# ruotianluo/ImageCaptioning.pytorch

Measured on AMD Instinct MI355X. Metric: captions/sec/node (UpDown SCST, bs10xsample_n5, 36x2048 feats), higher is better.
Workload: dtype f32; 1 GPU; UpDown SCST (BASELINE configs[2]): per-GPU batch 10 x train_sample_n 5, 36x2048 bottom-up feats, R=E=1000 A=512, vocab 9487, seq_len 20, references packed+cooked + greedy baseline + CIDEr-D + RewardCriterion + BPTT + clip 0.1 + Adam; rotating_batches=4, global_batch=10, seq_len=20, parallelism=dp1 (flat fp32 gradient, no collective)

## Files before the change

### imagecaptioning/pytorch_amd/csrc/attention.hip

```cpp
#include "capmi_common.h"
#include "profile.h"
#include <hip/hip_ext.h>
#include "../../../include/capmi.h"

using namespace capmi;

namespace {

constexpr int NMAX = 8;
constexpr int ATT_THREADS = 512;

__device__ __forceinline__ bool decode_block(int B, int chunks, int &b, int &chunk) {
    const int id = blockIdx.x;
    const int xcd = id & 7, slot = id >> 3;
    b = (slot / chunks) * 8 + xcd;
    chunk = slot % chunks;
    return b < B;
}
inline int grid_blocks(int B, int chunks) { return ((B + 7) / 8) * 8 * chunks; }
inline int pick_rpb(int B, int n) {
    int rpb = (int)(((long long)B * n) / 256);
    if (rpb < 1) rpb = 1;
    if (rpb > n) rpb = n;
    if (rpb > NMAX) rpb = NMAX;
// ... 677 lines not shown

constexpr int KCH = 12;
constexpr int DATT_T = 128;
__global__ __launch_bounds__(DATT_T) void attn_datt_kernel(const float *__restrict__ d_ctx_all, int ld_dctx,
                                                          const float *__restrict__ alpha_all, float *__restrict__ d_att,
                                                          int T, int N, int n, int K, int R) {
    const int b = blockIdx.x, kc = blockIdx.y * KCH;
    const int r = blockIdx.z * DATT_T + threadIdx.x;
    const int total = T * n;
    extern __shared__ float s_al[];
    for (int i = threadIdx.x; i < total * KCH; i += DATT_T) {
        const int row_i = i / KCH, q = i - row_i * KCH;
        const size_t row = (size_t)(row_i / n) * N + b * n + (row_i % n);
        s_al[i] = (kc + q < K) ? alpha_all[row * K + kc + q] : 0.f;
    }
    __syncthreads();
    if (r >= R) return;
    float acc[KCH];
#pragma unroll
    for (int q = 0; q < KCH; ++q) acc[q] = 0.f;
    for (int i0 = 0; i0 < total; i0 += 4) {
        float d[4];
#pragma unroll
        for (int u = 0; u < 4; ++u) {
            const int i = min(i0 + u, total - 1);
            const size_t row = (size_t)(i / n) * N + b * n + (i % n);
            d[u] = (i0 + u < total) ? d_ctx_all[row * ld_dctx + r] : 0.f;
        }
#pragma unroll
        for (int u = 0; u < 4; ++u) {
            const float *al = s_al + min(i0 + u, total - 1) * KCH;
#pragma unroll
            for (int q = 0; q < KCH; ++q) acc[q] += al[q] * d[u];
        }
    }
#pragma unroll
    for (int q = 0; q < KCH; ++q)
        if (kc + q < K) d_att[((size_t)b * K + kc + q) * R + r] = acc[q];
}

template <int KB>
__global__ void attn_dpatt_kernel(const float *__restrict__ att_h_all, const float *__restrict__ d_e_all,
                                  const float *__restrict__ p_att, const float *__restrict__ w,
                                  float *__restrict__ d_p_att, float *__restrict__ d_w, float *__restrict__ dw_part, int T, int N,
                                  int n, int K, int A) {
    const int kblocks = (K + KB - 1) / KB;
    const int b = blockIdx.x / kblocks, k0 = (blockIdx.x % kblocks) * KB;
    const int total = T * n;
    for (int a = threadIdx.x; a < A; a += blockDim.x) {
        float p[KB], acc[KB], accw[KB];
#pragma unroll
        for (int q = 0; q < KB; ++q) {
            p[q] = p_att[((size_t)b * K + min(k0 + q, K - 1)) * A + a];
            acc[q] = accw[q] = 0.f;
        }
        for (int i0 = 0; i0 < total; i0 += 8) {
            float de[8][KB], ah[8];
#pragma unroll
            for (int u = 0; u < 8; ++u) {
                const int i = min(i0 + u, total - 1);
                const size_t row = (size_t)(i / n) * N + b * n + (i % n);
#pragma unroll
                for (int q = 0; q < KB; ++q) de[u][q] = d_e_all[row * K + min(k0 + q, K - 1)];
                ah[u] = att_h_all[row * A + a];
            }
#pragma unroll
            for (int u = 0; u < 8; ++u)
                if (i0 + u < total) {
#pragma unroll
                    for (int q = 0; q < KB; ++q) {
                        const float th = tanh_f(p[q] + ah[u]);
                        acc[q] += de[u][q] * (1.f - th * th);
                        accw[q] += de[u][q] * th;
                    }
                }
        }
#pragma unroll
        for (int q = 0; q < KB; ++q) {
            if (k0 + q >= K) break;
            d_p_att[((size_t)b * K + k0 + q) * A + a] = w[a] * acc[q];
            if (dw_part) dw_part[((size_t)b * K + k0 + q) * A + a] = accw[q];
            else atomicAdd(&d_w[a], accw[q]);
        }
    }
}

__global__ void sum_all_kernel(const float *__restrict__ in, size_t live, size_t slab, size_t count, float *__restrict__ out) {
    __shared__ float scratch[32];
    float s = 0.f;
    const size_t stride = blockDim.x;
    const bool dense = slab == live;
    for (size_t i0 = threadIdx.x; i0 < count; i0 += 8 * stride) {
        float v[8];
#pragma unroll
        for (int u = 0; u < 8; ++u) {
            const size_t i = i0 + u * stride;
            v[u] = i < count ? in[dense ? i : (i / live) * slab + i % live] : 0.f;
        }
#pragma unroll
        for (int u = 0; u < 8; ++u) s += v[u];
    }
    s = block_sum(s, scratch);
    if (threadIdx.x == 0) out[0] = s;
}

}

extern "C" {

static int attention_fwd_launch(const float *att_h, int h_splits, int64_t h_stride, const float *h_bias, float *att_h_out,
                                const float *p_att, const float *att, const float *mask, const float *w, const float *b,
                                float *ctx, float *alpha, int B, int n, int K, int A, int R, const int32_t *row_img, int N,
                                void *stream, unsigned char *pl_ctx = nullptr) {
    if (!att_h || !p_att || !att || !w || !ctx || !alpha || B <= 0 || K <= 0 || A <= 0 || R <= 0) return CAPMI_EINVAL;
    if (row_img ? N <= 0 : n <= 0) return CAPMI_EINVAL;
    if (!row_img) N = B * n;
    if (pl_ctx && N > 64) return CAPMI_EINVAL;
    const size_t lds = ((size_t)NMAX * (A > 1024 ? A : 1024) + (size_t)NMAX * K) * sizeof(float);
    if (lds > 64 * 1024) return CAPMI_EINVAL;
    const double abytes = 4.0 * ((double)B * K * (A + R) + (double)N * (A + R + K));
    const int rpb = row_img ? 1 : pick_rpb_fwd(B, n), chunks = row_img ? 1 : (n + rpb - 1) / rpb;
    hipEvent_t e0, e1;
    static const int env_v2 = capmi::research("CAPMI_ATT_V2", 1);
    const bool al16 = ((reinterpret_cast<uintptr_t>(att_h) | reinterpret_cast<uintptr_t>(p_att) | reinterpret_cast<uintptr_t>(att) |
                        reinterpret_cast<uintptr_t>(w) | reinterpret_cast<uintptr_t>(ctx) | reinterpret_cast<uintptr_t>(h_bias) |
                        reinterpret_cast<uintptr_t>(att_h_out)) & 15) == 0;
    if (env_v2 && al16 && rpb <= 2 && (row_img ? N : grid_blocks(B, chunks)) <= 256 && K <= V2_KMAX && A % 4 == 0 && A >= 4 && A <= 512 && R % 4 == 0 && R >= 4 && R <= 1024 &&
        h_splits <= 16 && (h_stride & 3) == 0) {
        const size_t lds2 = ((size_t)rpb * 1024 + (size_t)rpb * V2_KMAX + (size_t)4 * rpb * 512) * sizeof(float);
        const bool prof = capmi_prof::take_events(CAPMI_PROF_ATTENTION_FWD, &e0, &e1, abytes, (double)N * K * (2.0 * A + 2.0 * R));
        const int gx = row_img ? N : grid_blocks(B, chunks);
        static const int env_cs = capmi::research("CAPMI_ATT_CS", 4);
        const int cs = (env_cs == 2 || env_cs == 4) && gx * env_cs <= 256 ? env_cs : 1;
        const dim3 grid(gx, cs);
#define CAPMI_ATT_V2(NR_, CS_)                                                                                              \
        if (prof) hipExtLaunchKernelGGL((attention_fwd_v2_kernel<NR_, CS_>), grid, dim3(ATT_THREADS), lds2, (hipStream_t)stream, e0, \
                                        e1, 0, att_h, p_att, att, mask, w, b, ctx, alpha, B, n, rpb, chunks, K, A, R, row_img,  \
                                        h_splits, (size_t)h_stride, h_bias, att_h_out, pl_ctx);                                \
        else hipLaunchKernelGGL((attention_fwd_v2_kernel<NR_, CS_>), grid, dim3(ATT_THREADS), lds2, (hipStream_t)stream, att_h, p_att, \
                                att, mask, w, b, ctx, alpha, B, n, rpb, chunks, K, A, R, row_img, h_splits, (size_t)h_stride,   \
                                h_bias, att_h_out, pl_ctx)
        if (rpb == 1) {
            if (cs == 4) { CAPMI_ATT_V2(1, 4); } else if (cs == 2) { CAPMI_ATT_V2(1, 2); } else { CAPMI_ATT_V2(1, 1); }
        } else {
            if (cs == 4) { CAPMI_ATT_V2(2, 4); } else if (cs == 2) { CAPMI_ATT_V2(2, 2); } else { CAPMI_ATT_V2(2, 1); }
        }
#undef CAPMI_ATT_V2
        CAPMI_CHECK_LAUNCH();
        return 0;
    }
    if (capmi_prof::take_events(CAPMI_PROF_ATTENTION_FWD, &e0, &e1, abytes, (double)N * K * (2.0 * A + 2.0 * R)))
        hipExtLaunchKernelGGL(attention_fwd_kernel, dim3(row_img ? N : grid_blocks(B, chunks)), dim3(ATT_THREADS), lds,
                              (hipStream_t)stream, e0, e1, 0, att_h, p_att, att, mask, w, b, ctx, alpha, B, n, rpb, chunks, K,
                              A, R, row_img, h_splits, (size_t)h_stride, h_bias, att_h_out, pl_ctx);
    else
        hipLaunchKernelGGL(attention_fwd_kernel, dim3(row_img ? N : grid_blocks(B, chunks)), dim3(ATT_THREADS), lds,
                           (hipStream_t)stream, att_h, p_att, att, mask, w, b, ctx, alpha, B, n, rpb, chunks, K, A, R, row_img,
                           h_splits, (size_t)h_stride, h_bias, att_h_out, pl_ctx);
    CAPMI_CHECK_LAUNCH();
    return 0;
}

int capmi_attention_fwd(const float *att_h, const float *p_att, const float *att, const float *mask, const float *w,
                        const float *b, float *ctx, float *alpha, int B, int n, int K, int A, int R,
                        const int32_t *row_img, int N, void *stream) {
    return attention_fwd_launch(att_h, 0, 0, nullptr, nullptr, p_att, att, mask, w, b, ctx, alpha, B, n, K, A, R, row_img, N,
// ... 12 lines not shown
int capmi_attention_fwd_partial_pl(const float *h_partial, int h_splits, int64_t h_stride, const float *h_bias,
                                   float *att_h_out, const float *p_att, const float *att, const float *mask, const float *w,
                                   const float *b, float *ctx, float *alpha, int B, int n, int K, int A, int R,
                                   const int32_t *row_img, int N, void *ctx_planes, void *stream) {
    if (h_splits < 1) return CAPMI_EINVAL;
    return attention_fwd_launch(h_partial, h_splits, h_stride, h_bias, att_h_out, p_att, att, mask, w, b, ctx, alpha, B, n, K,
                                A, R, row_img, N, stream, static_cast<unsigned char *>(ctx_planes));
}

static int attention_bwd_launch(const float *d_ctx, int ld_dctx, const float *x_slabs, int x_splits, int64_t x_stride, int x_cols,
                                float *x_out, const float *att_h, const float *alpha, const float *p_att, const float *att,
                                const float *w, float *d_att_h, float *d_e, int B, int n, int K, int A, int R,
                                const int32_t *row_img, int N, void *stream) {
    if (!att_h || !alpha || !p_att || !att || !w || !d_att_h || !d_e || B <= 0) return CAPMI_EINVAL;
    if (row_img ? N <= 0 : n <= 0) return CAPMI_EINVAL;
    if (!row_img) N = B * n;
    const size_t lds = ((size_t)NMAX * ((R + 3) & ~3) + (size_t)NMAX * K) * sizeof(float);
    if (lds > 64 * 1024) return CAPMI_EINVAL;
    const int rpb = row_img ? 1 : pick_rpb(B, n), chunks = row_img ? 1 : (n + rpb - 1) / rpb;
    static const int env_v2 = capmi::research("CAPMI_ATT_BWD_V2", 1);
    if (env_v2 && rpb == 1 && K <= BW2_KMAX && A <= ATT_THREADS && R % 4 == 0 && R <= 1024 &&
        (reinterpret_cast<uintptr_t>(att) & 15) == 0 && (!x_slabs || (x_cols - R) % 4 == 0)) {
        int roles = 1;
        if (x_slabs && x_cols > R) {
            roles = 1 + (x_cols - R + 1023) / 1024;
            if (roles > 4) roles = 4;
        }
        hipLaunchKernelGGL(attention_bwd_v2_kernel, dim3(row_img ? N : grid_blocks(B, chunks), roles), dim3(ATT_THREADS),
                           (size_t)(R + K) * sizeof(float), (hipStream_t)stream, d_ctx, ld_dctx, att_h, alpha, p_att, att, w,
                           d_att_h, d_e, B, n, chunks, K, A, R, row_img, x_slabs, x_splits, (size_t)x_stride, x_cols, x_out);
        CAPMI_CHECK_LAUNCH();
        return 0;
    }
    hipLaunchKernelGGL(attention_bwd_kernel, dim3(row_img ? N : grid_blocks(B, chunks)), dim3(ATT_THREADS), lds,
                       (hipStream_t)stream, d_ctx, ld_dctx, att_h, alpha, p_att, att, w, d_att_h, d_e, B, n, rpb, chunks, K,
                       A, R, row_img, x_slabs, x_splits, (size_t)x_stride, x_cols, x_out);
    CAPMI_CHECK_LAUNCH();
    return 0;
}

int capmi_attention_bwd(const float *d_ctx, int ld_dctx, const float *att_h, const float *alpha, const float *p_att,
                        const float *att, const float *mask, const float *w, float *d_att_h, float *d_e, int B, int n,
                        int K, int A, int R, const int32_t *row_img, int N, void *stream) {
    (void)mask;
    if (!d_ctx || ld_dctx < R) return CAPMI_EINVAL;
    return attention_bwd_launch(d_ctx, ld_dctx, nullptr, 0, 0, 0, nullptr, att_h, alpha, p_att, att, w, d_att_h, d_e, B, n, K, A,
                                R, row_img, N, stream);
}

int capmi_attention_bwd_partial(const float *x_slabs, int x_splits, int64_t x_stride, int x_cols, float *x_out,
                                const float *att_h, const float *alpha, const float *p_att, const float *att,
                                const float *w, float *d_att_h, float *d_e, int B, int n, int K, int A, int R,
                                const int32_t *row_img, int N, void *stream) {
    if (!x_slabs || !x_out || x_splits < 1 || x_cols < R) return CAPMI_EINVAL;
    if ((x_cols & 3) || (x_stride & 3) || ((reinterpret_cast<uintptr_t>(x_slabs) | reinterpret_cast<uintptr_t>(x_out)) & 15)) {
        const int rows = row_img ? N : B * n;
        if (x_stride != (int64_t)rows * x_cols) return CAPMI_EINVAL;
        const int rc = capmi_splitk_reduce(x_slabs, x_splits, x_out, x_cols, rows, x_cols, nullptr, nullptr, nullptr, 1, nullptr, 0,
                                           0, stream);
        if (rc) return rc;
        return attention_bwd_launch(x_out, x_cols, nullptr, 0, 0, 0, nullptr, att_h, alpha, p_att, att, w, d_att_h, d_e, B, n, K, A,
                                    R, row_img, N, stream);
    }
    return attention_bwd_launch(x_out, x_cols, x_slabs, x_splits, x_stride, x_cols, x_out, att_h, alpha, p_att, att, w, d_att_h,
                                d_e, B, n, K, A, R, row_img, N, stream);
}

int capmi_attention_bwd_batched(const float *d_ctx_all, int ld_dctx, const float *att_h_all, const float *alpha_all,
                                const float *d_e_all, const float *p_att, const float *w, float *d_att,
                                float *d_p_att, float *d_w, float *d_b, int T, int B, int n, int N_stride, int K, int A,
                                int R, void *stream) {
    return capmi_attention_bwd_batched_ws(d_ctx_all, ld_dctx, att_h_all, alpha_all, d_e_all, p_att, w, d_att, d_p_att, d_w, d_b, T,
                                          B, n, N_stride, K, A, R, nullptr, stream);
}

int capmi_attention_bwd_batched_ws(const float *d_ctx_all, int ld_dctx, const float *att_h_all, const float *alpha_all,
                                   const float *d_e_all, const float *p_att, const float *w, float *d_att,
                                   float *d_p_att, float *d_w, float *d_b, int T, int B, int n, int N_stride, int K, int A,
                                   int R, float *dw_partial, void *stream) {
    if (!d_ctx_all || !att_h_all || !alpha_all || !d_e_all || !p_att || !w || !d_att || !d_p_att || !d_b) return CAPMI_EINVAL;
    if (!d_w && !dw_partial) return CAPMI_EINVAL;
    hipStream_t st = (hipStream_t)stream;
    const int N = N_stride > 0 ? N_stride : B * n;
    hipLaunchKernelGGL(attn_datt_kernel, dim3(B, (K + KCH - 1) / KCH, (R + DATT_T - 1) / DATT_T), dim3(DATT_T),
                       (size_t)T * n * KCH * sizeof(float), st, d_ctx_all, ld_dctx, alpha_all, d_att, T, N, n, K, R);
    CAPMI_CHECK_LAUNCH();
    if (!dw_partial) {
        hipError_t e = hipMemsetAsync(d_w, 0, (size_t)A * sizeof(float), st);
        if (e != hipSuccess) return (int)e;
    }
    if ((B * ((K + 3) / 4)) >= 512)
        hipLaunchKernelGGL(attn_dpatt_kernel<4>, dim3(B * ((K + 3) / 4)), dim3(A >= 512 ? 512 : 256), 0, st, att_h_all, d_e_all, p_att, w,
                           d_p_att, d_w, dw_partial, T, N, n, K, A);
    else
        hipLaunchKernelGGL(attn_dpatt_kernel<1>, dim3(B * K), dim3(A >= 512 ? 512 : 256), 0, st, att_h_all, d_e_all, p_att, w,
                           d_p_att, d_w, dw_partial, T, N, n, K, A);
    CAPMI_CHECK_LAUNCH();
    hipLaunchKernelGGL(sum_all_kernel, dim3(1), dim3(1024), 0, st, d_e_all, (size_t)B * n * K, (size_t)N * K,
                       (size_t)T * B * n * K, d_b);
    CAPMI_CHECK_LAUNCH();
    return 0;
}

}

#include "host_common.h"

namespace {

constexpr uint64_t TILE_STREAM = 0x74696c65ULL;
constexpr int SSG = 4;

struct TileDrop {
    const float *mask;
    float p, scale;
    uint64_t seed;
    uint64_t row0;
    int on;
};

inline TileDrop tile_drop(const capmi_tile_drop *d) {
    TileDrop t{};
    if (d && (d->mask || d->p > 0.f)) {
        t.on = 1;
        t.mask = d->mask;
        t.p = d->p;
        t.scale = 1.f / (1.f - d->p);
        t.seed = d->seed;
        t.row0 = (uint64_t)d->row0;
    }
    return t;
}

template <int V>
__device__ __forceinline__ void ldv(const float *__restrict__ p, float (&o)[V]) {
    if constexpr (V == 4) {
        const f32x4 t = *reinterpret_cast<const f32x4 *>(p);
        o[0] = t[0]; o[1] = t[1]; o[2] = t[2]; o[3] = t[3];
    } else {
        o[0] = p[0];
    }
}

template <int V>
__device__ __forceinline__ void tile_keep(const TileDrop &td, const Philox &ph, uint64_t row, int kk, int a, int K1, int A,
                                          float (&m)[V]) {
    if (td.mask) {
        ldv<V>(td.mask + (row * K1 + kk) * (uint64_t)A + a, m);
        return;
    }
    const uint64_t idx = ((td.row0 + row) * K1 + kk) * (uint64_t)A + a;
    uint32_t o[4];
    ph.gen(idx >> 2, TILE_STREAM, o);
    if constexpr (V == 4) {
#pragma unroll
        for (int e = 0; e < 4; ++e) m[e] = (u01(o[e]) < td.p) ? 0.f : td.scale;
    } else {
        const uint32_t x = (idx & 2) ? ((idx & 1) ? o[3] : o[2]) : ((idx & 1) ? o[1] : o[0]);
        m[0] = (u01(x) < td.p) ? 0.f : td.scale;
    }
}

__device__ __forceinline__ float slab_sum8(const float *__restrict__ p, int splits, size_t stride) {
    float v = 0.f;
    for (int s0 = 0; s0 < splits; s0 += 8) {
        float part[8];
#pragma unroll
        for (int u = 0; u < 8; ++u) part[u] = (s0 + u < splits) ? p[(size_t)(s0 + u) * stride] : 0.f;
        v += ((part[0] + part[1]) + (part[2] + part[3])) + ((part[4] + part[5]) + (part[6] + part[7]));
    }
    return v;
}

template <int V>
__device__ __forceinline__ void sentinel_scores(const float *__restrict__ pb, const float *__restrict__ w, float bias,
// ... 464 lines not shown
```

### imagecaptioning/pytorch_amd/csrc/capmi_common.h

```cpp
#pragma once
#include <hip/hip_runtime.h>
#include <stdint.h>
#include <stdio.h>
#include <stdlib.h>

#define CAPMI_WAVE 64

#define CAPMI_CHECK_LAUNCH()                      \
    do {                                          \
        hipError_t e__ = hipGetLastError();       \
        if (e__ != hipSuccess) return (int)e__;   \
    } while (0)

typedef float f32x4 __attribute__((ext_vector_type(4)));
typedef float f32x16 __attribute__((ext_vector_type(16)));

namespace capmi {

template <int CTRL>
__device__ __forceinline__ float dpp_f(float v) {
    return __builtin_bit_cast(float, __builtin_amdgcn_update_dpp(0, __builtin_bit_cast(int, v), CTRL, 0xF, 0xF, true));
}
template <int CTRL>
__device__ __forceinline__ int dpp_i(int v) { return __builtin_amdgcn_update_dpp(0, v, CTRL, 0xF, 0xF, true); }
// ... 8 lines not shown
    return (lane_f(v, 0) + lane_f(v, 16)) + (lane_f(v, 32) + lane_f(v, 48));
}
__device__ __forceinline__ float wave_max(float v) {
    v = fmaxf(v, dpp_f<DPP_XOR1>(v));
    v = fmaxf(v, dpp_f<DPP_XOR2>(v));
    v = fmaxf(v, dpp_f<DPP_HALF_MIRROR>(v));
    v = fmaxf(v, dpp_f<DPP_ROW_MIRROR>(v));
    return fmaxf(fmaxf(lane_f(v, 0), lane_f(v, 16)), fmaxf(lane_f(v, 32), lane_f(v, 48)));
}
__device__ __forceinline__ double wave_sum_d(double v) {
#pragma unroll
    for (int o = 32; o > 0; o >>= 1) v += __shfl_xor(v, o, 64);
    return v;
}

__device__ __forceinline__ float block_sum(float v, float *scratch) {
    v = wave_sum(v);
    const int lane = threadIdx.x & 63, wid = threadIdx.x >> 6, nw = (blockDim.x + 63) >> 6;
    __syncthreads();
    if (lane == 0) scratch[wid] = v;
    __syncthreads();
    float r = 0.f;
    for (int i = 0; i < nw; ++i) r += scratch[i];
    return r;
}
__device__ __forceinline__ float block_max(float v, float *scratch) {
    v = wave_max(v);
    const int lane = threadIdx.x & 63, wid = threadIdx.x >> 6, nw = (blockDim.x + 63) >> 6;
    __syncthreads();
    if (lane == 0) scratch[wid] = v;
    __syncthreads();
    float r = scratch[0];
    for (int i = 1; i < nw; ++i) r = fmaxf(r, scratch[i]);
    return r;
}

__device__ __forceinline__ float rcp_f(float x) { return __builtin_amdgcn_rcpf(x); }
__device__ __forceinline__ float tanh_f(float x) {
    const float ax = fabsf(x);
    const float e = __expf(-2.0f * ax);
    const float t = (1.0f - e) * rcp_f(1.0f + e);
    return copysignf(t, x);
}
__device__ __forceinline__ float sigmoid_f(float x) {
    const float e = __expf(-fabsf(x));
    const float s = rcp_f(1.0f + e);
    return x >= 0.f ? s : 1.0f - s;
}

struct Philox {
    uint32_t k0, k1;
    __device__ __forceinline__ Philox(uint64_t seed) : k0((uint32_t)seed), k1((uint32_t)(seed >> 32)) {}
    __device__ __forceinline__ static void round(uint32_t (&c)[4], uint32_t a, uint32_t b) {
        const uint64_t p0 = (uint64_t)0xD2511F53u * c[0];
        const uint64_t p1 = (uint64_t)0xCD9E8D57u * c[2];
        const uint32_t n0 = (uint32_t)(p1 >> 32) ^ c[1] ^ a;
        const uint32_t n1 = (uint32_t)p1;
        const uint32_t n2 = (uint32_t)(p0 >> 32) ^ c[3] ^ b;
        const uint32_t n3 = (uint32_t)p0;
        c[0] = n0; c[1] = n1; c[2] = n2; c[3] = n3;
    }
    __device__ __forceinline__ void gen(uint64_t ctr_lo, uint64_t ctr_hi, uint32_t (&out)[4]) const {
        uint32_t c[4] = {(uint32_t)ctr_lo, (uint32_t)(ctr_lo >> 32), (uint32_t)ctr_hi, (uint32_t)(ctr_hi >> 32)};
        uint32_t a = k0, b = k1;
#pragma unroll
        for (int i = 0; i < 10; ++i) {
            round(c, a, b);
            a += 0x9E3779B9u;
            b += 0xBB67AE85u;
        }
        out[0] = c[0]; out[1] = c[1]; out[2] = c[2]; out[3] = c[3];
    }
};
__device__ __forceinline__ uint64_t epoch_seed(uint64_t seed, const uint64_t *__restrict__ epoch) {
    return epoch ? seed + 0x9E3779B97F4A7C15ull * *epoch : seed;
}
__device__ __forceinline__ float u01(uint32_t x) { return ((float)(x >> 8) + 0.5f) * (1.0f / 16777216.0f); }

const uint64_t *rng_epoch();
static inline int knob(const char *name, int dflt) {
    const char *e = getenv(name);
    return e ? atoi(e) : dflt;
}
#ifdef CAPMI_VARIANTS
static inline int research(const char *name, int dflt) {
    const char *e = getenv(name);
    if (e) fprintf(stderr, "*** capmi (variants build): research switch %s=%s ***\n", name, e);
    return e ? atoi(e) : dflt;
}
static inline int ablate_env(const char *name) {
    const char *e = getenv(name);
    int v = e ? atoi(e) : 0;
    if (v)
        fprintf(stderr, "\n*** capmi: %s=%d -- PROFILING ABLATION ACTIVE, kernel results are deliberately incomplete; "
                        "unset it for any real run ***\n\n", name, v);
    return v;
}
#else
static inline constexpr int research(const char *, int dflt) { return dflt; }
static inline constexpr int ablate_env(const char *) { return 0; }
#endif
}

#define CAPMI_PL_CHUNK_BYTES 12288
#define CAPMI_PL_PLANE_BYTES 4096

namespace capmi {
__device__ __forceinline__ uint32_t f2u(float x) { return __builtin_bit_cast(uint32_t, x); }
__device__ __forceinline__ float u2f(uint32_t x) { return __builtin_bit_cast(float, x); }
__device__ __forceinline__ size_t pl_offset(int row, int k) {
    const int kk = k & 31;
    return (size_t)(k >> 5) * CAPMI_PL_CHUNK_BYTES + row * 64 + ((((kk >> 3) ^ (row >> 2)) & 3) << 4) + ((kk & 7) << 1);
}
__device__ __forceinline__ void pl_store1(unsigned char *pl, int row, int k, float x) {
    const uint32_t h = f2u(x) & 0xffff0000u;
    const float r1 = x - u2f(h);
    const uint32_t m = f2u(r1) & 0xffff0000u;
    const uint32_t l = f2u(r1 - u2f(m));
    unsigned char *o = pl + pl_offset(row, k);
    *reinterpret_cast<unsigned short *>(o) = (unsigned short)(h >> 16);
    *reinterpret_cast<unsigned short *>(o + CAPMI_PL_PLANE_BYTES) = (unsigned short)(m >> 16);
    *reinterpret_cast<unsigned short *>(o + 2 * CAPMI_PL_PLANE_BYTES) = (unsigned short)(l >> 16);
}
__device__ __forceinline__ void pl_store4(unsigned char *pl, int row, int k, f32x4 v) {
    typedef unsigned int u32x2_ __attribute__((ext_vector_type(2)));
    uint32_t h[4], m[4], l[4];
#pragma unroll
    for (int e = 0; e < 4; ++e) {
        h[e] = f2u(v[e]) & 0xffff0000u;
        const float r1 = v[e] - u2f(h[e]);
        m[e] = f2u(r1) & 0xffff0000u;
        l[e] = f2u(r1 - u2f(m[e]));
    }
    unsigned char *o = pl + pl_offset(row, k);
    *reinterpret_cast<u32x2_ *>(o) = u32x2_{(h[0] >> 16) | (h[1] & 0xffff0000u), (h[2] >> 16) | (h[3] & 0xffff0000u)};
    *reinterpret_cast<u32x2_ *>(o + CAPMI_PL_PLANE_BYTES) = u32x2_{(m[0] >> 16) | (m[1] & 0xffff0000u), (m[2] >> 16) | (m[3] & 0xffff0000u)};
    *reinterpret_cast<u32x2_ *>(o + 2 * CAPMI_PL_PLANE_BYTES) = u32x2_{(l[0] >> 16) | (l[1] & 0xffff0000u), (l[2] >> 16) | (l[3] & 0xffff0000u)};
}
}
```

### imagecaptioning/pytorch_amd/csrc/embed_bwd_det.h

```cpp
#pragma once
#include "capmi_common.h"

namespace capmi {

constexpr int EBD_THREADS = 1024, EBD_WAVES = EBD_THREADS / 64;
constexpr int EBD_MAX_ROWS = 14336;

template <typename G>
__device__ __forceinline__ void embed_bwd_det_body(const int64_t *__restrict__ tok, int T, int tok_ld, int rows, int D,
                                                   float *__restrict__ dE, const G &g) {
    extern __shared__ unsigned char ebd_smem[];
    int *list = reinterpret_cast<int *>(ebd_smem);
    f32x4 *part = reinterpret_cast<f32x4 *>(ebd_smem + (size_t)((rows + 3) & ~3) * sizeof(int));
    __shared__ int s_cnt[EBD_WAVES];
    const int i = blockIdx.x, tid = threadIdx.x, wave = tid >> 6, lane = tid & 63;
    const int64_t my = tok[(size_t)(i / T) * tok_ld + (i % T)];
    int n = 0;
    for (int base = 0; base < rows; base += EBD_THREADS) {
        const int j = base + tid;
        const bool m = j < rows && tok[(size_t)(j / T) * tok_ld + (j % T)] == my;
        const unsigned long long b = __ballot(m);
        if (lane == 0) s_cnt[wave] = __popcll(b);
        __syncthreads();
        int before = n;
        for (int w = 0; w < wave; ++w) before += s_cnt[w];
        if (m) list[before + __popcll(b & ((1ull << lane) - 1ull))] = j;
#pragma unroll
        for (int w = 0; w < EBD_WAVES; ++w) n += s_cnt[w];
        __syncthreads();
        if (n > 0 && list[0] != i) return;
    }
    const int c = (blockIdx.y * 64 + lane) * 4;
    const int per = (n + EBD_WAVES - 1) / EBD_WAVES, lo = wave * per, hi = min(n, lo + per);
    f32x4 acc = {0.f, 0.f, 0.f, 0.f};
    if (c < D) {
        int k = lo;
        for (; k + 8 <= hi; k += 8) {
            f32x4 a[8];
#pragma unroll
            for (int u = 0; u < 8; ++u) a[u] = g((size_t)list[k + u], c);
#pragma unroll
            for (int u = 0; u < 8; ++u) acc += a[u];
        }
        for (; k < hi; ++k) acc += g((size_t)list[k], c);
    }
    part[wave * 64 + lane] = acc;
    __syncthreads();
    if (wave == 0 && c < D) {
        f32x4 s = part[lane];
#pragma unroll
        for (int w = 1; w < EBD_WAVES; ++w) s += part[w * 64 + lane];
        f32x4 *o = reinterpret_cast<f32x4 *>(dE + (size_t)my * D + c);
        *o = *o + s;
    }
}

static inline size_t embed_bwd_det_lds(int rows) { return (size_t)((rows + 3) & ~3) * sizeof(int) + EBD_WAVES * 64 * sizeof(f32x4); }

}
```

### imagecaptioning/pytorch_amd/csrc/pointwise.hip

```cpp
#include <cstdlib>
#include "host_common.h"
#include "profile.h"
#include "embed_bwd_det.h"

using namespace capmi;

#include <atomic>
static std::atomic<const uint64_t *> g_rng_epoch{nullptr};
namespace capmi {
const uint64_t *rng_epoch() { return g_rng_epoch.load(std::memory_order_relaxed); }
}

namespace {

__global__ void embed_fwd_kernel(const int64_t *__restrict__ it, int it_stride, int64_t *__restrict__ it_save,
                                 const float *__restrict__ E, const float *__restrict__ mask, float *__restrict__ x,
                                 int N, int Ed, int relu, unsigned char *__restrict__ pl) {
    const size_t total = (size_t)N * Ed;
    for (size_t i = (size_t)blockIdx.x * blockDim.x + threadIdx.x; i < total; i += (size_t)gridDim.x * blockDim.x) {
        const int r = (int)(i / Ed), c = (int)(i % Ed);
        const int64_t tok = it[(size_t)r * it_stride];
        if (it_save && c == 0) it_save[r] = tok;
        float v = E[(size_t)tok * Ed + c];
        if (relu) v = fmaxf(v, 0.f);
// ... 580 lines not shown
        const size_t q1 = q0 + stride;
        const bool two = q1 < quads;
        const size_t q1c = two ? q1 : q0;
        f32x4 gg[2], pp[2], mm[2], vv[2];
        if (NT) {
            gg[0] = __builtin_nontemporal_load(g4 + q0); gg[1] = __builtin_nontemporal_load(g4 + q1c);
            mm[0] = __builtin_nontemporal_load(m4 + q0); mm[1] = __builtin_nontemporal_load(m4 + q1c);
            vv[0] = __builtin_nontemporal_load(v4 + q0); vv[1] = __builtin_nontemporal_load(v4 + q1c);
        } else {
            gg[0] = g4[q0]; gg[1] = g4[q1c]; mm[0] = m4[q0]; mm[1] = m4[q1c]; vv[0] = v4[q0]; vv[1] = v4[q1c];
        }
        pp[0] = p4[q0]; pp[1] = p4[q1c];
#pragma unroll
        for (int u = 0; u < 2; ++u)
#pragma unroll
            for (int k = 0; k < 4; ++k) {
                float x = gg[u][k] * gscale;
                if (clip > 0.f) x = fminf(fmaxf(x, -clip), clip);
                if (wd != 0.f) x += wd * pp[u][k];
                mm[u][k] = b1 * mm[u][k] + (1.f - b1) * x;
                vv[u][k] = b2 * vv[u][k] + (1.f - b2) * x * x;
                pp[u][k] -= step_size * mm[u][k] / (sqrtf(vv[u][k]) / bc2_sqrt + eps);
            }
        p4[q0] = pp[0];
        if (NT) { __builtin_nontemporal_store(mm[0], m4 + q0); __builtin_nontemporal_store(vv[0], v4 + q0); }
        else { m4[q0] = mm[0]; v4[q0] = vv[0]; }
        if (two) {
            p4[q1] = pp[1];
            if (NT) { __builtin_nontemporal_store(mm[1], m4 + q1); __builtin_nontemporal_store(vv[1], v4 + q1); }
            else { m4[q1] = mm[1]; v4[q1] = vv[1]; }
        }
    }
}

__global__ void step_advance_kernel(capmi_step_state *st, float b1, float b2) {
    st->epoch += 1;
    const int step = st->adam_step + 1;
    st->adam_step = step;
    st->bc1 = (float)(1.0 - pow((double)b1, (double)step));
    st->bc2_sqrt = (float)sqrt(1.0 - pow((double)b2, (double)step));
}
__global__ void step_set_lr_kernel(capmi_step_state *st, float lr) { st->lr = lr; }

__global__ void scst_advantage_kernel(const double *__restrict__ scores, int N, int n, float *__restrict__ reward,
                                      float *__restrict__ mean_out) {
    __shared__ float scratch[32];
    float s = 0.f;
    for (int r = threadIdx.x; r < N; r += blockDim.x) {
        const float a = (float)(scores[r] - scores[N + r / n]);
        reward[r] = a;
        s += a;
    }
    if (mean_out) {
        s = block_sum(s, scratch);
        if (threadIdx.x == 0) mean_out[0] = s / (float)N;
    }
}

}

extern "C" {

int capmi_embed_fwd_pl(const int64_t *it, int it_stride, int64_t *it_save, const float *E, const float *mask, float *x,
                       int N, int Edim, int relu, void *x_planes, void *stream) {
    if (!it || !E || !x || N <= 0 || Edim <= 0 || it_stride < 1 || (x_planes && N > 64)) return CAPMI_EINVAL;
    hipLaunchKernelGGL(embed_fwd_kernel, dim3(grid_for((size_t)N * Edim)), dim3(256), 0, (hipStream_t)stream, it,
                       it_stride, it_save, E, mask, x, N, Edim, relu, static_cast<unsigned char *>(x_planes));
    CAPMI_CHECK_LAUNCH();
    return 0;
}

int capmi_embed_fwd(const int64_t *it, int it_stride, int64_t *it_save, const float *E, const float *mask, float *x,
                    int N, int Edim, int relu, void *stream) {
    return capmi_embed_fwd_pl(it, it_stride, it_save, E, mask, x, N, Edim, relu, nullptr, stream);
}

int capmi_embed_bwd(const int64_t *it, const float *dx, const float *x_saved, const float *mask, float *dE, int rows,
                    int Edim, int relu, void *stream) {
    if (!it || !dx || !dE || rows <= 0 || Edim <= 0 || (relu && !x_saved)) return CAPMI_EINVAL;
    static const int det = capmi::knob("CAPMI_EMBED_BWD_DET", 1);
    if (det && Edim % 4 == 0 && rows <= EBD_MAX_ROWS &&
        ((reinterpret_cast<uintptr_t>(dx) | reinterpret_cast<uintptr_t>(x_saved) | reinterpret_cast<uintptr_t>(mask) |
          reinterpret_cast<uintptr_t>(dE)) & 15) == 0) {
        hipLaunchKernelGGL(embed_bwd_det_kernel, dim3(rows, (Edim + 255) / 256), dim3(EBD_THREADS), embed_bwd_det_lds(rows),
                           (hipStream_t)stream, it, rows, Edim, dE, EmbedGrad{dx, x_saved, mask, Edim, relu});
        CAPMI_CHECK_LAUNCH();
        return 0;
    }
    hipLaunchKernelGGL(embed_bwd_kernel, dim3(grid_for((size_t)rows * Edim)), dim3(256), 0, (hipStream_t)stream, it, dx,
                       x_saved, mask, dE, rows, Edim, relu);
    CAPMI_CHECK_LAUNCH();
    return 0;
}

int capmi_lstm_cell_fwd_pl(const float *partial, int splits, const float *b_ih, const float *b_hh, const float *row_bias,
                           int row_bias_div, const int32_t *row_bias_idx, const float *c_prev, float *h, float *c,
                           float *gates_act, const float *out_mask, float *h_drop, int N, int R, void *h_planes,
                           void *h_drop_planes, void *stream) {
    return capmi_lstm_cell_fwd_pl2(partial, splits, nullptr, 0, b_ih, b_hh, row_bias, row_bias_div, row_bias_idx, c_prev, h, c,
                                   gates_act, out_mask, h_drop, N, R, h_planes, h_drop_planes, stream);
}

int capmi_lstm_cell_fwd_pl2(const float *partial, int splits, const float *partial2, int splits2, const float *b_ih,
                            const float *b_hh, const float *row_bias, int row_bias_div, const int32_t *row_bias_idx,
                            const float *c_prev, float *h, float *c, float *gates_act, const float *out_mask, float *h_drop,
                            int N, int R, void *h_planes, void *h_drop_planes, void *stream) {
    if (!partial || splits < 1 || !c_prev || !h || !c || N <= 0 || R <= 0 || splits2 < 0 || (splits2 > 0 && !partial2))
        return CAPMI_EINVAL;
    if (splits2 == 0) partial2 = nullptr;
    if ((h_planes || h_drop_planes) && N > 64) return CAPMI_EINVAL;
    unsigned char *pl_h = static_cast<unsigned char *>(h_planes), *pl_hd = static_cast<unsigned char *>(h_drop_planes);
    const int rbd = row_bias_div > 0 ? row_bias_div : 1;
    if (R % 4 == 0 && aligned16(partial, partial2, b_ih, b_hh, row_bias, c_prev, h, c, gates_act, out_mask, h_drop)) {
        const int quads = N * (R / 4);
        hipLaunchKernelGGL(lstm_cell_fwd_vec_kernel, dim3((quads + 63) / 64), dim3(64), 0, (hipStream_t)stream, partial, splits,
                           b_ih, b_hh, row_bias, rbd, row_bias_idx, c_prev, h, c, gates_act, out_mask, h_drop, N, R, pl_h, pl_hd,
                           partial2, splits2);
        CAPMI_CHECK_LAUNCH();
        return 0;
    }
    hipLaunchKernelGGL(lstm_cell_fwd_kernel, dim3(grid_for((size_t)N * R)), dim3(256), 0, (hipStream_t)stream, partial,
                       splits, b_ih, b_hh, row_bias, rbd, row_bias_idx, c_prev, h, c, gates_act, out_mask, h_drop, N, R, pl_h,
                       pl_hd, partial2, splits2);
    CAPMI_CHECK_LAUNCH();
    return 0;
}

int capmi_lstm_cell_fwd(const float *partial, int splits, const float *b_ih, const float *b_hh, const float *row_bias,
                        int row_bias_div, const int32_t *row_bias_idx, const float *c_prev, float *h, float *c, float *gates_act,
                        const float *out_mask, float *h_drop, int N, int R, void *stream) {
    return capmi_lstm_cell_fwd_pl(partial, splits, b_ih, b_hh, row_bias, row_bias_div, row_bias_idx, c_prev, h, c, gates_act,
                                  out_mask, h_drop, N, R, nullptr, nullptr, stream);
}

int capmi_lstm_cell_bwd_partial(const float *dh_a, int ld_a, const float *dh_a_mask, const float *dh_b, int ld_b,
                                int b_splits, int64_t b_stride, const float *dh_c, int ld_c, int c_splits,
                                int64_t c_stride, const float *dc_next, const float *gates_act, const float *c_prev,
                                const float *c_new, float *d_gates, float *dc_prev, int N, int R, void *stream) {
    return capmi_lstm_cell_bwd_partial_pl(dh_a, ld_a, dh_a_mask, dh_b, ld_b, b_splits, b_stride, dh_c, ld_c, c_splits, c_stride,
                                          dc_next, gates_act, c_prev, c_new, d_gates, dc_prev, N, R, nullptr, stream);
}

int capmi_lstm_cell_bwd_partial_pl(const float *dh_a, int ld_a, const float *dh_a_mask, const float *dh_b, int ld_b,
                                   int b_splits, int64_t b_stride, const float *dh_c, int ld_c, int c_splits,
                                   int64_t c_stride, const float *dc_next, const float *gates_act, const float *c_prev,
                                   const float *c_new, float *d_gates, float *dc_prev, int N, int R, void *d_gates_planes,
                                   void *stream) {
    if (!gates_act || !c_prev || !c_new || !d_gates || !dc_prev || N <= 0 || R <= 0) return CAPMI_EINVAL;
    if ((dh_b && b_splits < 1) || (dh_c && c_splits < 1) || (d_gates_planes && N > 64)) return CAPMI_EINVAL;
    unsigned char *pl_dg = static_cast<unsigned char *>(d_gates_planes);
    if (R % 4 == 0 && ld_a % 4 == 0 && ld_b % 4 == 0 && ld_c % 4 == 0 && b_stride % 4 == 0 && c_stride % 4 == 0 &&
        aligned16(dh_a, dh_a_mask, dh_b, dh_c, dc_next, gates_act, c_prev, c_new, d_gates, dc_prev)) {
        const int quads = N * (R / 4);
        hipLaunchKernelGGL(lstm_cell_bwd_vec_kernel, dim3((quads + 63) / 64), dim3(64), 0, (hipStream_t)stream, dh_a, ld_a,
                           dh_a_mask, dh_b, ld_b, b_splits, (size_t)b_stride, dh_c, ld_c, c_splits, (size_t)c_stride, dc_next,
                           gates_act, c_prev, c_new, d_gates, dc_prev, N, R, pl_dg);
        CAPMI_CHECK_LAUNCH();
        return 0;
    }
    hipLaunchKernelGGL(lstm_cell_bwd_kernel, dim3(grid_for((size_t)N * R)), dim3(256), 0, (hipStream_t)stream, dh_a,
                       ld_a, dh_a_mask, dh_b, ld_b, b_splits, (size_t)b_stride, dh_c, ld_c, c_splits, (size_t)c_stride,
                       dc_next, gates_act, c_prev, c_new, d_gates, dc_prev, N, R, pl_dg);
    CAPMI_CHECK_LAUNCH();
    return 0;
}

// ... 190 lines not shown
```

### imagecaptioning/pytorch_amd/csrc/transformer.hip

```cpp
#include "host_common.h"
#include "embed_bwd_det.h"

using namespace capmi;

namespace {

__global__ void layernorm_fwd_kernel(const float *__restrict__ x, const float *__restrict__ a, const float *__restrict__ b,
                                     float *__restrict__ y, float *__restrict__ mean, float *__restrict__ inv, int M, int D,
                                     float eps) {
    const int lane = threadIdx.x & 63, wid = threadIdx.x >> 6, nw = blockDim.x >> 6;
    for (int r = blockIdx.x * nw + wid; r < M; r += gridDim.x * nw) {
        const float *xr = x + (size_t)r * D;
        float s = 0.f;
        for (int c = lane; c < D; c += 64) s += xr[c];
        const float mu = wave_sum(s) / D;
        float v = 0.f;
        for (int c = lane; c < D; c += 64) {
            const float d = xr[c] - mu;
            v += d * d;
        }
        const float sd = sqrtf(wave_sum(v) / (D - 1));
        const float iv = 1.f / (sd + eps);
        for (int c = lane; c < D; c += 64) y[(size_t)r * D + c] = a[c] * (xr[c] - mu) * iv + b[c];
        if (lane == 0) {
// ... 1093 lines not shown
                  const float *drop, float *dq, float *dk_out, float *dv_out, int dkv_ld, int dkv_stride, int accumulate,
                  int Nq, int q_per_kv, int Tq, int Tk, int h, int dk, void *stream) {
    return capmi_mha_bwd_s(d_o, q, 0, k, v, ldkv, kstride, p, drop, dq, 0, dk_out, dv_out, dkv_ld, dkv_stride, accumulate, Nq, q_per_kv,
                           Tq, Tk, h, dk, stream);
}

int capmi_mha_bwd_s(const float *d_o, const float *q, int qstride, const float *k, const float *v, int ldkv, int kstride,
                    const float *p, const float *drop, float *dq, int dq_stride, float *dk_out, float *dv_out, int dkv_ld,
                    int dkv_stride, int accumulate, int Nq, int q_per_kv, int Tq, int Tk, int h, int dk, void *stream) {
    return capmi_mha_bwd_slabs(d_o, 1, 0, h * dk, q, qstride, k, v, ldkv, kstride, p, drop, dq, dq_stride, dk_out, dv_out, dkv_ld,
                               dkv_stride, accumulate, Nq, q_per_kv, Tq, Tk, h, dk, stream);
}

int capmi_mha_bwd_slabs(const float *d_o, int do_splits, int64_t do_stride, int do_ld, const float *q, int qstride, const float *k,
                        const float *v, int ldkv, int kstride, const float *p, const float *drop, float *dq, int dq_stride,
                        float *dk_out, float *dv_out, int dkv_ld, int dkv_stride, int accumulate, int Nq, int q_per_kv, int Tq,
                        int Tk, int h, int dk, void *stream) {
    if (do_splits < 1 || do_ld < h * dk || do_ld % 4 || (do_splits > 1 && (do_stride % 4 || do_stride < (int64_t)Nq * Tq * do_ld)))
        return CAPMI_EINVAL;
    if (qstride <= 0) qstride = h * dk;
    if (dq_stride <= 0) dq_stride = h * dk;
    if (qstride % 4 || dq_stride % 4) return CAPMI_EINVAL;
    if (kstride <= 0) kstride = h * dk;
    if (dkv_stride <= 0) dkv_stride = h * dk;
    if (dkv_ld <= 0) dkv_ld = Tk * dkv_stride;
    if (!d_o || !q || !k || !v || !p || !dq || !dk_out || !dv_out || Nq <= 0 || q_per_kv <= 0 || Nq % q_per_kv)
        return CAPMI_EINVAL;
    if (dk % 4 || ldkv % 4 || kstride % 4 || dkv_ld % 4 || dkv_stride % 4 ||
        ((reinterpret_cast<uintptr_t>(d_o) | reinterpret_cast<uintptr_t>(q) | reinterpret_cast<uintptr_t>(k) |
          reinterpret_cast<uintptr_t>(v) | reinterpret_cast<uintptr_t>(dq) | reinterpret_cast<uintptr_t>(dk_out) |
          reinterpret_cast<uintptr_t>(dv_out)) & 15))
        return CAPMI_EINVAL;
    const int64_t fixed_b = (int64_t)4 * Tk * (dk + 4), per_b = (int64_t)2 * (dk + 4) + 3 * (Tk + 1) + 1;
    const int64_t wgs = (int64_t)(Nq / q_per_kv) * h;
    const int CH = mha_chunk(q_per_kv * Tq, fixed_b, per_b);
    const size_t lds = (size_t)(fixed_b + (int64_t)CH * per_b) * sizeof(float);
    if (lds > 160 * 1024) return CAPMI_EINVAL;
    static bool attr_b = false;
    if (!attr_b) {
        (void)hipFuncSetAttribute(reinterpret_cast<const void *>(&mha_bwd_kernel<MHA_T_BIG>), hipFuncAttributeMaxDynamicSharedMemorySize, 160 * 1024);
        (void)hipFuncSetAttribute(reinterpret_cast<const void *>(&mha_bwd_kernel<MHA_T_MAX>), hipFuncAttributeMaxDynamicSharedMemorySize, 160 * 1024);
        (void)hipFuncSetAttribute(reinterpret_cast<const void *>(&mha_bwd_kernel<MHA_T_BIG, true>), hipFuncAttributeMaxDynamicSharedMemorySize, 160 * 1024);
        (void)hipFuncSetAttribute(reinterpret_cast<const void *>(&mha_bwd_kernel<MHA_T_MAX, true>), hipFuncAttributeMaxDynamicSharedMemorySize, 160 * 1024);
        attr_b = true;
    }
    const int threads = mha_threads(CH, Tk, wgs);
    mha_sync_ablation();
    if (do_splits > 1 || do_ld != h * dk) {
        if (threads > MHA_T_BIG)
            hipLaunchKernelGGL((mha_bwd_kernel<MHA_T_MAX, true>), dim3(Nq / q_per_kv, h), dim3(threads), lds, (hipStream_t)stream, d_o, q, k, v,
                               ldkv, kstride, p, drop, dq, dk_out, dv_out, dkv_ld, dkv_stride, accumulate, q_per_kv, Tq, Tk, h, dk, CH,
                               qstride, dq_stride, mha_on_mfma(CH), do_ld, do_splits, (size_t)do_stride);
        else
            hipLaunchKernelGGL((mha_bwd_kernel<MHA_T_BIG, true>), dim3(Nq / q_per_kv, h), dim3(threads), lds, (hipStream_t)stream, d_o, q, k, v,
                               ldkv, kstride, p, drop, dq, dk_out, dv_out, dkv_ld, dkv_stride, accumulate, q_per_kv, Tq, Tk, h, dk, CH,
                               qstride, dq_stride, mha_on_mfma(CH), do_ld, do_splits, (size_t)do_stride);
    } else if (threads > MHA_T_BIG)
        hipLaunchKernelGGL(mha_bwd_kernel<MHA_T_MAX>, dim3(Nq / q_per_kv, h), dim3(threads), lds, (hipStream_t)stream, d_o, q, k, v, ldkv,
                           kstride, p, drop, dq, dk_out, dv_out, dkv_ld, dkv_stride, accumulate, q_per_kv, Tq, Tk, h, dk, CH, qstride,
                           dq_stride, mha_on_mfma(CH), do_ld, do_splits, (size_t)do_stride);
    else
        hipLaunchKernelGGL(mha_bwd_kernel<MHA_T_BIG>, dim3(Nq / q_per_kv, h), dim3(threads), lds, (hipStream_t)stream, d_o, q, k, v, ldkv,
                           kstride, p, drop, dq, dk_out, dv_out, dkv_ld, dkv_stride, accumulate, q_per_kv, Tq, Tk, h, dk, CH, qstride,
                           dq_stride, mha_on_mfma(CH), do_ld, do_splits, (size_t)do_stride);
    CAPMI_CHECK_LAUNCH();
    return 0;
}

int capmi_embed_pe_fwd(const int64_t *tok, int tok_ld, const float *E, const float *pe, const float *drop, float *x, int N,
                       int T, int D, int pos0, void *stream) {
    if (!tok || !E || !pe || !x || N <= 0 || T <= 0 || D <= 0 || pos0 < 0) return CAPMI_EINVAL;
    hipLaunchKernelGGL(embed_pe_fwd_kernel, dim3(grid_for((size_t)N * T * D, 256, 4096)), dim3(256), 0, (hipStream_t)stream, tok, tok_ld,
                       E, pe, drop, x, N, T, D, pos0, sqrtf((float)D));
    CAPMI_CHECK_LAUNCH();
    return 0;
}

int capmi_embed_pe_bwd(const int64_t *tok, int tok_ld, const float *dx, const float *drop, float *dE, int N, int T, int D,
                       void *stream) {
    if (!tok || !dx || !dE || N <= 0 || T <= 0 || D <= 0) return CAPMI_EINVAL;
    static const int det = capmi::knob("CAPMI_EMBED_BWD_DET", 1);
    if (det && D % 4 == 0 && (int64_t)N * T <= capmi::EBD_MAX_ROWS &&
        ((reinterpret_cast<uintptr_t>(dx) | reinterpret_cast<uintptr_t>(drop) | reinterpret_cast<uintptr_t>(dE)) & 15) == 0) {
        hipLaunchKernelGGL(embed_pe_bwd_det_kernel, dim3(N * T, (D + 255) / 256), dim3(capmi::EBD_THREADS),
                           capmi::embed_bwd_det_lds(N * T), (hipStream_t)stream, tok, T, tok_ld, N * T, D, dE,
                           EmbedPeGrad{dx, drop, D, sqrtf((float)D)});
        CAPMI_CHECK_LAUNCH();
        return 0;
    }
    hipLaunchKernelGGL(embed_pe_bwd_kernel, dim3(grid_for((size_t)N * T * D, 256, 4096)), dim3(256), 0, (hipStream_t)stream, tok, tok_ld,
                       dx, drop, dE, N, T, D, sqrtf((float)D));
    CAPMI_CHECK_LAUNCH();
    return 0;
}

int capmi_glu_fwd(const float *pre, const float *mask, const float *residual, float *out, int M, int R, void *stream) {
    if (!pre || !out || M <= 0 || R <= 0) return CAPMI_EINVAL;
    hipLaunchKernelGGL(glu_fwd_kernel, dim3(grid_for((size_t)M * R, 256, 4096)), dim3(256), 0, (hipStream_t)stream, pre, mask, residual, out,
                       M, R);
    CAPMI_CHECK_LAUNCH();
    return 0;
}

int capmi_glu_fwd_fused(const float *slabs, int splits, int64_t stride, const float *bias, float *pre, float *out,
                        const float *mask_a, float *out_a, void *planes_a, const float *mask_b, float *out_b, void *planes_b,
                        int M, int R, void *stream) {
    if (!slabs || !pre || !out || splits < 1 || M <= 0 || R <= 0 || R % 4 || stride % 4) return CAPMI_EINVAL;
    if ((planes_a || planes_b) && M > 64) return CAPMI_EINVAL;
    if ((planes_a && !out_a) || (planes_b && !out_b)) return CAPMI_EINVAL;
    if ((reinterpret_cast<uintptr_t>(slabs) | reinterpret_cast<uintptr_t>(bias) | reinterpret_cast<uintptr_t>(pre) |
         reinterpret_cast<uintptr_t>(out) | reinterpret_cast<uintptr_t>(mask_a) | reinterpret_cast<uintptr_t>(out_a) |
         reinterpret_cast<uintptr_t>(mask_b) | reinterpret_cast<uintptr_t>(out_b) | reinterpret_cast<uintptr_t>(planes_a) |
         reinterpret_cast<uintptr_t>(planes_b)) & 15)
        return CAPMI_EINVAL;
    hipLaunchKernelGGL(glu_fwd_fused_kernel, dim3(grid_for((size_t)M * (R / 4), 256, 4096)), dim3(256), 0, (hipStream_t)stream, slabs, splits,
                       (size_t)stride, bias, pre, out, mask_a, out_a, static_cast<unsigned char *>(planes_a), mask_b, out_b,
                       static_cast<unsigned char *>(planes_b), M, R);
    CAPMI_CHECK_LAUNCH();
    return 0;
}

int capmi_glu_bwd(const float *d_out, const float *mask, const float *pre, float *d_pre, int M, int R, void *stream) {
    return capmi_glu_bwd_add(d_out, mask, nullptr, 0, 0, nullptr, pre, d_pre, M, R, stream);
}

int capmi_glu_bwd_add(const float *d_out, const float *mask, const float *add_slabs, int add_splits, int64_t add_stride,
                      const float *add_mask, const float *pre, float *d_pre, int M, int R, void *stream) {
    if (!d_out || !pre || !d_pre || M <= 0 || R <= 0) return CAPMI_EINVAL;
    if (add_slabs && (add_splits < 1 || (add_splits > 1 && add_stride < (int64_t)M * R))) return CAPMI_EINVAL;
    hipLaunchKernelGGL(glu_bwd_kernel, dim3(grid_for((size_t)M * R, 256, 4096)), dim3(256), 0, (hipStream_t)stream, d_out, mask, pre, d_pre,
                       M, R, add_slabs, add_splits, (size_t)add_stride, add_mask);
    CAPMI_CHECK_LAUNCH();
    return 0;
}

int capmi_split_halves(const float *slabs, int splits, int64_t stride, const float *mask_lo, const float *mask_hi, float *out_lo,
                       float *out_hi, int M, int R, void *stream) {
    if (!slabs || !out_lo || !out_hi || splits < 1 || M <= 0 || R <= 0) return CAPMI_EINVAL;
    hipLaunchKernelGGL(split_halves_kernel, dim3(grid_for((size_t)M * 2 * R, 256, 4096)), dim3(256), 0, (hipStream_t)stream, slabs, splits,
                       (size_t)stride, mask_lo, mask_hi, out_lo, out_hi, M, R);
    CAPMI_CHECK_LAUNCH();
    return 0;
}

int capmi_meanpool_fwd(const float *x, const float *mask, float *mean, int B, int K, int D, void *stream) {
    if (!x || !mean || B <= 0 || K <= 0 || D <= 0) return CAPMI_EINVAL;
    hipLaunchKernelGGL(meanpool_fwd_kernel, dim3(B), dim3(256), 0, (hipStream_t)stream, x, mask, mean, K, D);
    CAPMI_CHECK_LAUNCH();
    return 0;
}

int capmi_meanpool_bwd(const float *dmean, const float *mask, float *dx, int accumulate, int B, int K, int D, void *stream) {
    if (!dmean || !dx || B <= 0 || K <= 0 || D <= 0) return CAPMI_EINVAL;
    hipLaunchKernelGGL(meanpool_bwd_kernel, dim3(grid_for((size_t)B * K * D, 256, 4096)), dim3(256), 0, (hipStream_t)stream, dmean, mask, dx,
                       accumulate, B, K, D);
    CAPMI_CHECK_LAUNCH();
    return 0;
}

int capmi_caption_stats(const float *seq_logp, const int64_t *seq, int N, int L, int V1, float *scratch, float *entropy, float *perplexity,
                        void *stream) {
    if (!seq_logp || !seq || !scratch || !entropy || !perplexity || N <= 0 || L <= 0 || V1 <= 0 || V1 > 32 * 1024) return CAPMI_EINVAL;
    float *ent_t = scratch, *sel_t = scratch + (size_t)N * L;
#define CAPMI_CS(NE_) hipLaunchKernelGGL(caption_step_stats_kernel<NE_>, dim3(N * L), dim3(1024), 0, (hipStream_t)stream, seq_logp, seq, V1, ent_t, sel_t)
    if (V1 <= 10 * 1024) CAPMI_CS(10);
    else if (V1 <= 16 * 1024) CAPMI_CS(16);
// ... 23 lines not shown
```

Baseline: 12590 captions/s.

## Add register-blocked attention backward kernels for small-batch dAtt and dPatt

Adds attn_datt2_kernel, which uses 64-thread blocks and preloads 100 d_ctx values per thread into registers with 32-bit offset arithmetic, reading alpha from LDS as float4. It also adds attn_dpatt2_kernel, which broadcasts d_e through readlane instead of loading it per thread. Both are picked by default for small problem sizes, and CAPMI_TAIL_V1 switches back to the old kernels. Separately, the embedding-backward deterministic kernels now opt in to a larger dynamic LDS limit. The point is to lower memory-latency and indexing overhead in the attention backward tail, at the cost of higher register pressure and a partly unfused FMA path kept to preserve numerics.

```diff
diff --git a/imagecaptioning/pytorch_amd/csrc/attention.hip b/imagecaptioning/pytorch_amd/csrc/attention.hip
--- a/imagecaptioning/pytorch_amd/csrc/attention.hip
+++ b/imagecaptioning/pytorch_amd/csrc/attention.hip
@@ -783,6 +783,112 @@
             if (dw_part) dw_part[((size_t)b * K + k0 + q) * A + a] = accw[q];
             else atomicAdd(&d_w[a], accw[q]);
         }
+    }
+}
+
+constexpr int DATT2_T = 64, DATT2_RC = 100;
+constexpr int DATT_FUSED = 10;
+__device__ __forceinline__ float mul_add_unfused(float a, float b, float c) {
+    float p = a * b;
+    asm("" : "+v"(p));
+    return c + p;
+}
+__global__ __launch_bounds__(DATT2_T) void attn_datt2_kernel(const float *__restrict__ d_ctx_all, int ld_dctx,
+                                                            const float *__restrict__ alpha_all, float *__restrict__ d_att,
+                                                            int T, int N, int n, int K, int R) {
+    const int b = blockIdx.x, kc = blockIdx.y * KCH;
+    const int r = blockIdx.z * DATT2_T + threadIdx.x;
+    const int total = T * n;
+    const uint32_t rc = (uint32_t)min(r, R - 1);
+    const uint32_t ld = (uint32_t)ld_dctx, tstep = (uint32_t)(N - n + 1) * ld;
+    extern __shared__ __attribute__((aligned(16))) float s_al2[];
+    float *s_al = s_al2;
+    static_assert(KCH % 4 == 0, "alpha rows are read as float4");
+    float acc[KCH];
+#pragma unroll
+    for (int q = 0; q < KCH; ++q) acc[q] = 0.f;
+    for (int i0 = 0; i0 < total; i0 += DATT2_RC) {
+        float d[DATT2_RC];
+        const int tq = i0 / n;
+        int jr = i0 - tq * n;
+        uint32_t off = ((uint32_t)tq * N + b * n + jr) * ld + rc;
+#pragma unroll
+        for (int u = 0; u < DATT2_RC; ++u) {
+            d[u] = d_ctx_all[off];
+            const bool more = i0 + u + 1 < total, wrap = jr + 1 == n;
+            off += more ? (wrap ? tstep : ld) : 0u;
+            jr = more ? (wrap ? 0 : jr + 1) : jr;
+        }
+        if (i0 == 0) {
+            const int padded = (total + DATT2_RC - 1) / DATT2_RC * DATT2_RC;
+            for (int row_i = threadIdx.x; row_i < padded; row_i += DATT2_T) {
+                const int rl = min(row_i, total - 1);
+                const size_t row = (size_t)(rl / n) * N + b * n + (rl % n);
+#pragma unroll
+                for (int q = 0; q < KCH; ++q)
+                    s_al[row_i * KCH + q] = (kc + q < K && row_i < total) ? alpha_all[row * K + min(kc + q, K - 1)] : 0.f;
+            }
+            __syncthreads();
+        }
+        const f32x4 *al4 = reinterpret_cast<const f32x4 *>(s_al + i0 * KCH);
+#pragma unroll
+        for (int u = 0; u < DATT2_RC; ++u) {
+#pragma unroll
+            for (int q4 = 0; q4 < KCH / 4; ++q4) {
+                const f32x4 al = al4[u * (KCH / 4) + q4];
+#pragma unroll
+                for (int e = 0; e < 4; ++e) {
+                    const int q = q4 * 4 + e;
+                    acc[q] = q < DATT_FUSED ? __builtin_fmaf(al[e], d[u], acc[q]) : mul_add_unfused(al[e], d[u], acc[q]);
+                }
+            }
+        }
+    }
+    if (r >= R) return;
+#pragma unroll
+    for (int q = 0; q < KCH; ++q)
+        if (kc + q < K) d_att[((size_t)b * K + kc + q) * R + r] = acc[q];
+}
+
+constexpr int DPATT2_RC = 50;
+__global__ __launch_bounds__(512) void attn_dpatt2_kernel(const float *__restrict__ att_h_all, const float *__restrict__ d_e_all,
+                                                         const float *__restrict__ p_att, const float *__restrict__ w,
+                                                         float *__restrict__ d_p_att, float *__restrict__ d_w,
+                                                         float *__restrict__ dw_part, int T, int N, int n, int K, int A) {
+    const int b = blockIdx.x / K, k = blockIdx.x % K;
+    const int total = T * n;
+    const uint32_t tstep = (uint32_t)(N - n + 1) * (uint32_t)A;
+    for (int a0 = 0; a0 < A; a0 += blockDim.x) {
+        const int a = min(a0 + (int)threadIdx.x, A - 1);
+        const float p = p_att[((size_t)b * K + k) * A + a];
+        float acc = 0.f, accw = 0.f;
+        for (int i0 = 0; i0 < total; i0 += DPATT2_RC) {
+            float ah[DPATT2_RC];
+            const int il = min(i0 + (int)(threadIdx.x & 63), total - 1);
+            const float de_l = d_e_all[((size_t)(il / n) * N + b * n + (il % n)) * K + k];
+            const int tq = i0 / n;
+            int jr = i0 - tq * n;
+            uint32_t off = ((uint32_t)tq * N + b * n + jr) * (uint32_t)A + a;
+#pragma unroll
+            for (int u = 0; u < DPATT2_RC; ++u) {
+                ah[u] = att_h_all[off];
+                const bool more = i0 + u + 1 < total, wrap = jr + 1 == n;
+                off += more ? (wrap ? tstep : (uint32_t)A) : 0u;
+                jr = more ? (wrap ? 0 : jr + 1) : jr;
+            }
+#pragma unroll
+            for (int u = 0; u < DPATT2_RC; ++u)
+                if (i0 + u < total) {
+                    const float de = capmi::u2f(__builtin_amdgcn_readlane(capmi::f2u(de_l), u));
+                    const float th = tanh_f(p + ah[u]);
+                    acc += de * (1.f - th * th);
+                    accw += de * th;
+                }
+        }
+        if (a0 + (int)threadIdx.x >= A) continue;
+        d_p_att[((size_t)b * K + k) * A + a] = w[a] * acc;
+        if (dw_part) dw_part[((size_t)b * K + k) * A + a] = accw;
+        else atomicAdd(&d_w[a], accw);
     }
 }
 
@@ -961,8 +1067,15 @@
     if (!d_w && !dw_partial) return CAPMI_EINVAL;
     hipStream_t st = (hipStream_t)stream;
     const int N = N_stride > 0 ? N_stride : B * n;
-    hipLaunchKernelGGL(attn_datt_kernel, dim3(B, (K + KCH - 1) / KCH, (R + DATT_T - 1) / DATT_T), dim3(DATT_T),
-                       (size_t)T * n * KCH * sizeof(float), st, d_ctx_all, ld_dctx, alpha_all, d_att, T, N, n, K, R);
+    const bool v1 = capmi::tail_v1();
+    const bool small_dctx = (uint64_t)T * N * (uint64_t)ld_dctx < (1ull << 30), small_atth = (uint64_t)T * N * (uint64_t)A < (1ull << 30);
+    const bool datt_small = (long)B * ((K + KCH - 1) / KCH) * ((R + DATT_T - 1) / DATT_T) <= 1024;
+    if (v1 || !small_dctx || !datt_small)
+        hipLaunchKernelGGL(attn_datt_kernel, dim3(B, (K + KCH - 1) / KCH, (R + DATT_T - 1) / DATT_T), dim3(DATT_T),
+                           (size_t)T * n * KCH * sizeof(float), st, d_ctx_all, ld_dctx, alpha_all, d_att, T, N, n, K, R);
+    else
+        hipLaunchKernelGGL(attn_datt2_kernel, dim3(B, (K + KCH - 1) / KCH, (R + DATT2_T - 1) / DATT2_T), dim3(DATT2_T),
+                           (size_t)((T * n + DATT2_RC - 1) / DATT2_RC * DATT2_RC) * KCH * sizeof(float), st, d_ctx_all, ld_dctx, alpha_all, d_att, T, N, n, K, R);
     CAPMI_CHECK_LAUNCH();
     if (!dw_partial) {
         hipError_t e = hipMemsetAsync(d_w, 0, (size_t)A * sizeof(float), st);
@@ -970,6 +1083,9 @@
     }
     if ((B * ((K + 3) / 4)) >= 512)
         hipLaunchKernelGGL(attn_dpatt_kernel<4>, dim3(B * ((K + 3) / 4)), dim3(A >= 512 ? 512 : 256), 0, st, att_h_all, d_e_all, p_att, w,
+                           d_p_att, d_w, dw_partial, T, N, n, K, A);
+    else if (!v1 && small_atth)
+        hipLaunchKernelGGL(attn_dpatt2_kernel, dim3(B * K), dim3(A >= 512 ? 512 : 256), 0, st, att_h_all, d_e_all, p_att, w,
                            d_p_att, d_w, dw_partial, T, N, n, K, A);
     else
         hipLaunchKernelGGL(attn_dpatt_kernel<1>, dim3(B * K), dim3(A >= 512 ? 512 : 256), 0, st, att_h_all, d_e_all, p_att, w,
diff --git a/imagecaptioning/pytorch_amd/csrc/capmi_common.h b/imagecaptioning/pytorch_amd/csrc/capmi_common.h
--- a/imagecaptioning/pytorch_amd/csrc/capmi_common.h
+++ b/imagecaptioning/pytorch_amd/csrc/capmi_common.h
@@ -114,6 +114,7 @@
     const char *e = getenv(name);
     return e ? atoi(e) : dflt;
 }
+static inline bool tail_v1() { return knob("CAPMI_TAIL_V1", 0) != 0; }
 #ifdef CAPMI_VARIANTS
 static inline int research(const char *name, int dflt) {
     const char *e = getenv(name);
diff --git a/imagecaptioning/pytorch_amd/csrc/embed_bwd_det.h b/imagecaptioning/pytorch_amd/csrc/embed_bwd_det.h
--- a/imagecaptioning/pytorch_amd/csrc/embed_bwd_det.h
+++ b/imagecaptioning/pytorch_amd/csrc/embed_bwd_det.h
@@ -57,4 +57,10 @@
 
 static inline size_t embed_bwd_det_lds(int rows) { return (size_t)((rows + 3) & ~3) * sizeof(int) + EBD_WAVES * 64 * sizeof(f32x4); }
 
+static inline void embed_bwd_det_lds_optin(const void *kernel, bool *done) {
+    if (*done) return;
+    (void)hipFuncSetAttribute(kernel, hipFuncAttributeMaxDynamicSharedMemorySize, (int)embed_bwd_det_lds(EBD_MAX_ROWS));
+    *done = true;
 }
+
+}
diff --git a/imagecaptioning/pytorch_amd/csrc/pointwise.hip b/imagecaptioning/pytorch_amd/csrc/pointwise.hip
--- a/imagecaptioning/pytorch_amd/csrc/pointwise.hip
+++ b/imagecaptioning/pytorch_amd/csrc/pointwise.hip
@@ -686,6 +686,8 @@
     if (det && Edim % 4 == 0 && rows <= EBD_MAX_ROWS &&
         ((reinterpret_cast<uintptr_t>(dx) | reinterpret_cast<uintptr_t>(x_saved) | reinterpret_cast<uintptr_t>(mask) |
           reinterpret_cast<uintptr_t>(dE)) & 15) == 0) {
+        static bool optin = false;
+        embed_bwd_det_lds_optin(reinterpret_cast<const void *>(&embed_bwd_det_kernel), &optin);
         hipLaunchKernelGGL(embed_bwd_det_kernel, dim3(rows, (Edim + 255) / 256), dim3(EBD_THREADS), embed_bwd_det_lds(rows),
                            (hipStream_t)stream, it, rows, Edim, dE, EmbedGrad{dx, x_saved, mask, Edim, relu});
         CAPMI_CHECK_LAUNCH();
diff --git a/imagecaptioning/pytorch_amd/csrc/transformer.hip b/imagecaptioning/pytorch_amd/csrc/transformer.hip
--- a/imagecaptioning/pytorch_amd/csrc/transformer.hip
+++ b/imagecaptioning/pytorch_amd/csrc/transformer.hip
@@ -1199,6 +1199,8 @@
     static const int det = capmi::knob("CAPMI_EMBED_BWD_DET", 1);
     if (det && D % 4 == 0 && (int64_t)N * T <= capmi::EBD_MAX_ROWS &&
         ((reinterpret_cast<uintptr_t>(dx) | reinterpret_cast<uintptr_t>(drop) | reinterpret_cast<uintptr_t>(dE)) & 15) == 0) {
+        static bool optin = false;
+        capmi::embed_bwd_det_lds_optin(reinterpret_cast<const void *>(&embed_pe_bwd_det_kernel), &optin);
         hipLaunchKernelGGL(embed_pe_bwd_det_kernel, dim3(N * T, (D + 255) / 256), dim3(capmi::EBD_THREADS),
                            capmi::embed_bwd_det_lds(N * T), (hipStream_t)stream, tok, T, tok_ld, N * T, D, dE,
                            EmbedPeGrad{dx, drop, D, sqrtf((float)D)});
```

After: 12700 captions/s, median of 6. No clear change (+0.9%).
